# facebookresearch/pytorch3d

Hardware: AMD Instinct MI355X
Metric: rasterized Mpix/s (fwd+bwd) at 512^2 faces_per_pixel=8 (higher is better)
Workload: dtype f32

## Files before the change

### pytorch3d_amd/csrc/raster_mesh.hip

```cpp
#include "binning.h"
#include "tile_map.h"
#include "chunk_order.h"
#include "p3d_geom.h"
#include "topk.h"

#include <stdio.h>
#include <stdlib.h>


namespace p3d {

namespace {

constexpr int kTile = 16;
constexpr int kStage = 256;
constexpr int kMeshPayload = 4;
constexpr int kSplitMaxTiles = 512;

constexpr int kFineWaves = 4;

struct MeshArgs {
  const float* face_verts;
  const int64_t* neighbor;
  const int64_t* mesh_first;
  const int64_t* mesh_count;
  BinCSR csr;
  int N, H, W, K;
  TileMap tm;
  float blur, sqrt_blur;
  int persp, clip, cull;
  int walk_plan;
  int64_t* p2f;
  float* zbuf;
  float* bary;
  float* dists;
  int* cover;
  int CY, CX;
  int* area_count;
  int* area_list;
  int list_by_plan;
  const int* overflow;
  int ties;
  unsigned long long* tie_words;
  int SY, SX;
};

typedef unsigned int u32x4 __attribute__((ext_vector_type(4)));
__device__ __forceinline__ void store16(void* p, unsigned a, unsigned b, unsigned c, unsigned d) {
  u32x4 v = {a, b, c, d};
  *reinterpret_cast<u32x4*>(p) = v;
}

template <int KT>
__device__ __forceinline__ void store_row(float* dst, const float (&v)[KT]) {
  if constexpr (KT % 4 == 0) {
#pragma unroll
    for (int k = 0; k < KT; k += 4) {
      float4 t;
      t.x = v[k];
      t.y = v[k + 1];
      t.z = v[k + 2];
      t.w = v[k + 3];
      *reinterpret_cast<float4*>(dst + k) = t;
    }
  } else if constexpr (KT == 2) {
    float2 t;
    t.x = v[0];
    t.y = v[1];
    *reinterpret_cast<float2*>(dst) = t;
  } else {
#pragma unroll
    for (int k = 0; k < KT; ++k) dst[k] = v[k];
  }
}

template <typename Queue, int KT, bool IN_REGS>
__device__ __forceinline__ void write_pixel(const MeshArgs& a, const Queue& q, int64_t opix) {
  static_assert(IN_REGS, "vector-row stores need the register queue");
  const int64_t base = opix * KT;
  float zv[KT], dv[KT], bv[3 * KT];
  long long iv[KT];
#pragma unroll
  for (int k = 0; k < KT; ++k) {
    const bool ok = q.valid(k);
    iv[k] = ok ? (long long)q.ix(k) : -1ll;
    zv[k] = ok ? q.zf(k) : -1.0f;
    dv[k] = ok ? q.pay(0, k) : -1.0f;
    bv[3 * k + 0] = ok ? q.pay(1, k) : -1.0f;
    bv[3 * k + 1] = ok ? q.pay(2, k) : -1.0f;
    bv[3 * k + 2] = ok ? q.pay(3, k) : -1.0f;
  }
  if constexpr (KT % 4 == 0) {
#pragma unroll
    for (int k = 0; k < KT; k += 4) {
      store16(a.zbuf + base + k, __float_as_uint(zv[k]), __float_as_uint(zv[k + 1]), __float_as_uint(zv[k + 2]),
                  __float_as_uint(zv[k + 3]));
      store16(a.dists + base + k, __float_as_uint(dv[k]), __float_as_uint(dv[k + 1]), __float_as_uint(dv[k + 2]),
                  __float_as_uint(dv[k + 3]));
    }
#pragma unroll
    for (int k = 0; k < 3 * KT; k += 4)
      store16(a.bary + base * 3 + k, __float_as_uint(bv[k]), __float_as_uint(bv[k + 1]), __float_as_uint(bv[k + 2]),
                  __float_as_uint(bv[k + 3]));
#pragma unroll
    for (int k = 0; k < KT; k += 2)
      store16(a.p2f + base + k, (unsigned)iv[k], (unsigned)(iv[k] >> 32), (unsigned)iv[k + 1], (unsigned)(iv[k + 1] >> 32));
  } else {
    store_row<KT>(a.zbuf + base, zv);
    store_row<KT>(a.dists + base, dv);
#pragma unroll
    for (int k = 0; k < 3 * KT; ++k) a.bary[base * 3 + k] = bv[k];
    if constexpr (KT % 2 == 0) {
      long long* ip = reinterpret_cast<long long*>(a.p2f + base);
#pragma unroll
      for (int k = 0; k < KT; k += 2) {
        longlong2 t;
        t.x = iv[k];
        t.y = iv[k + 1];
        *reinterpret_cast<longlong2*>(ip + k) = t;
      }
    } else {
#pragma unroll
      for (int k = 0; k < KT; ++k) a.p2f[base + k] = iv[k];
    }
  }
}

template <typename Queue, int KT, bool IN_REGS>
__device__ __forceinline__ void write_subtile_fill_patch(const MeshArgs& a, const Queue& q, bool have, int n, int sy0,
                                                         int sx0, int y_end, int x_end, int lane, bool pix_ok, int yi,
                                                         int xi) {
  const int H = a.H, W = a.W, K = a.K;
  const int rows = min(8, y_end - sy0), cols = min(8, x_end - sx0);
  const int seg = cols * K;
  const int64_t col0 = W - sx0 - cols;
  const bool patch = have;
  for (int r = 0; r < rows; ++r) {
    const int64_t px = ((int64_t)n * H + (H - 1 - (sy0 + r))) * W + col0;
    if ((K & 3) == 0) {
      const int q4 = seg >> 2;
      const float4 m1 = make_float4(-1.0f, -1.0f, -1.0f, -1.0f);
      longlong2 i1;
      i1.x = -1;
      i1.y = -1;
      float4* zb = reinterpret_cast<float4*>(a.zbuf + px * K);
      float4* db = reinterpret_cast<float4*>(a.dists + px * K);
      float4* bb = reinterpret_cast<float4*>(a.bary + px * K * 3);
      longlong2* ib = reinterpret_cast<longlong2*>(a.p2f + px * K);
      for (int e = lane; e < 3 * q4; e += 64) {
        bb[e] = m1;
        if (e < 2 * q4) ib[e] = i1;
        if (e < q4) {
          zb[e] = m1;
          db[e] = m1;
        }
      }
    } else {
      for (int e = lane; e < 3 * seg; e += 64) {
        a.bary[px * K * 3 + e] = -1.0f;
        if (e < seg) {
          a.p2f[px * K + e] = -1;
// ... 210 lines not shown
    const unsigned alo = (unsigned)__builtin_amdgcn_readlane((int)mlo, ci), ahi = (unsigned)__builtin_amdgcn_readlane((int)mhi, ci);
    unsigned long long inside = ((unsigned long long)ahi << 32) | (unsigned long long)alo;
    float zc = __int_as_float(__builtin_amdgcn_readlane(__float_as_int(zcv), ci));
    if constexpr (!GENERAL) {
      const unsigned long long free_of_a = __ballot(((mlo & alo) | (mhi & ahi)) == 0u) & cand;
      if (free_of_a) {
        const int cb = __builtin_ctzll(free_of_a);
        cand &= ~(1ull << cb);
        const unsigned long long in_b = ((unsigned long long)(unsigned)__builtin_amdgcn_readlane((int)mhi, cb) << 32) |
                                        (unsigned long long)(unsigned)__builtin_amdgcn_readlane((int)mlo, cb);
        const bool mine_is_b = __builtin_amdgcn_inverse_ballot_w64(in_b);
        const int jb = __builtin_amdgcn_readlane(oj, cb);
        const float zb = __int_as_float(__builtin_amdgcn_readlane(__float_as_int(zcv), cb));
        jj = mine_is_b ? jb : jj;
        zc = mine_is_b ? zb : zc;
        inside |= in_b;
      }
    }
    const bool in_box = __builtin_amdgcn_inverse_ballot_w64(inside);
    const bool too_deep = zc > q.kth_z(K);
    if (pix_ok && in_box && !too_deep) {
      const float kz0 = TIES ? q.kth_z(K) : 0.0f;
      const int ki0 = TIES ? q.kth_i(K) : 0;
      if constexpr (TIES && GENERAL) tie_z = INFINITY;
      const float4* rec = reinterpret_cast<const float4*>(reinterpret_cast<const char*>(s_rec) + __umul24((unsigned)jj, (unsigned)(kRecWords * sizeof(float4))));
      const float4 r0 = rec[0], r1 = rec[1], r2 = rec[2];
      const int f = __float_as_int(r2.y);
      FaceHit h;
      bool hit = false;
      {
        const double2 d0 = *reinterpret_cast<const double2*>(&rec[3]);
        const double2 d1 = *reinterpret_cast<const double2*>(&rec[4]);
        FaceRec fr;
        fr.v0 = mk3(r0.x, r0.y, r1.z);
        fr.v1 = mk3(r0.z, r0.w, r1.w);
        fr.v2 = mk3(r1.x, r1.y, r2.x);
        fr.rd_area = d0.x;
        fr.rd_l01 = d0.y;
        fr.rd_l02 = d1.x;
        fr.rd_l12 = d1.y;
        const float4 r5 = rec[5];
        const float2 r6 = *reinterpret_cast<const float2*>(&rec[6]);
        fr.d01 = mk2(r5.x, r5.y);
        fr.d12 = mk2(r5.z, r5.w);
        fr.d20 = mk2(r6.x, r6.y);
        const bool pcs = PC && !GENERAL;
        fr.wide = pcs ? false : __float_as_int(r2.w) != 0;
        const f3 bp = face_depth_rec(fr, p, pcs || persp, pcs || clip, &h);
        const bool adm = !(h.z < 0.0f) & q.admits(K, h.z, f);
        if constexpr (TIES && !GENERAL) {
          const bool ev = (h.z == kz0) & !adm;
          const int d = kz0 == tie_z ? min(tie_drop, f) : f;
          tie_drop = ev ? d : tie_drop;
          tie_z = ev ? kz0 : tie_z;
        }
        if (GENERAL || adm) hit = face_dist_rec<PC && !GENERAL>(fr, p, a.blur, bp, &h);
      }
      if (hit) {
        bool ins = true;
        if constexpr (GENERAL) {
          const int nb = __float_as_int(r2.z);
          if (nb != -1) {
            const int at = q.find(nb);
            if (at >= 0) {
              float queued;
              if constexpr (Queue::kPayload > 0) {
                queued = q.payload_at(0, at);
              } else {
                queued = recompute_face(a, nb, p, persp, clip).dist;
              }
              if (fabsf(h.dist) < fabsf(queued))
                q.erase(at);
              else
                ins = false;
            }
          }
        }
        if (ins && q.admits(K, h.z, f)) {
          if constexpr (Queue::kPayload > 0) {
            const float pl[kMeshPayload] = {h.dist, h.bary.x, h.bary.y, h.bary.z};
            q.insert(K, h.z, f, pl);
          } else {
            const float none[1] = {0.0f};
            q.insert(K, h.z, f, none);
          }
          if constexpr (TIES && !GENERAL) {
            const bool ev = (kz0 < INFINITY) & (q.kth_z(K) == kz0);
            const int d = kz0 == tie_z ? min(tie_drop, ki0) : ki0;
            tie_drop = ev ? d : tie_drop;
            tie_z = ev ? kz0 : tie_z;
          }
        }
      }
    }
  }
}

__device__ __forceinline__ void cover_mark(const MeshArgs& a, int n, int sy0, bool any, int yo, int xo, int lane) {
  unsigned long long rem = __ballot(any);
  const int wid = (yo >> 4) * a.CX + (xo >> 4);
  while (rem) {
    const int w0 = __builtin_amdgcn_readlane(wid, __builtin_ctzll(rem));
    const unsigned long long same = __ballot(any && wid == w0);
    unsigned bits = 0;
#pragma unroll
    for (int j = 0; j < 8; ++j)
      if ((same >> (8 * j)) & 0xffull) bits |= 1u << ((a.H - 1 - (sy0 + j)) & 15);
    rem &= ~same;
    if (lane == 0) {
      const int word = (n * a.CY) * a.CX + w0;
      if (a.area_list != nullptr && !a.list_by_plan) {
        const int before = atomicOr(a.cover + word, (int)bits);
        if (before == 0 && bits != 0u) a.area_list[atomicAdd(a.area_count, 1)] = word;
      } else {
        atomicOr(a.cover + word, (int)bits);
      }
    }
  }
}

__device__ __forceinline__ float uniform_f(float v) { return __int_as_float(__builtin_amdgcn_readfirstlane(__float_as_int(v))); }

struct StageLds {
  unsigned* pm;
  float pxy;
  unsigned valid_c, valid_r;
  float4 (*rec)[kRecWords];
  float* zc;
  int* order;
  float* qlow;
  ChunkOrderScratch* ord;
  int* wcnt;
};

struct TileRect {
  float x0, x1, y0, y1;
};

template <bool BINNED, bool PC = false>
__device__ __forceinline__ int stage_chunk(const MeshArgs& a, const StageLds& l, const TileRect& tile, int64_t src_base,
                                           int count, int base, int tid, bool cull, bool clip, bool prune, bool* general) {
  const int lane = tid & 63, w = tid >> 6;
  const int i = base + tid;
  bool keep = false;
  f3 v0, v1, v2;
  FaceSetup fs;
  int fid = -1, nb = -1;
  unsigned cm = 0, rm = 0;
  const bool has = i < count;
  fs.xlo = fs.xhi = fs.ylo = fs.yhi = 0.0f;
  fs.reject = true;
  if (has) {
    fid = BINNED ? a.csr.list[src_base + i] : (int)(src_base + i);
    const float* g = a.face_verts + (int64_t)fid * 9;
    nb = (int)a.neighbor[fid];
    v0 = mk3(g[0], g[1], g[2]);
    v1 = mk3(g[3], g[4], g[5]);
    v2 = mk3(g[6], g[7], g[8]);
    fs = face_setup(v0, v1, v2, a.sqrt_blur, cull);
  }
  int xb = 0, xa = 0, yb = 0, ya = 0;
  if (__ballot(has) != 0) {
#pragma unroll
    for (int c = 0; c < 16; ++c) {
      const float xs = __int_as_float(__builtin_amdgcn_readlane(__float_as_int(l.pxy), c));
      const float ys = __int_as_float(__builtin_amdgcn_readlane(__float_as_int(l.pxy), 16 + c));
      xb += xs < fs.xlo ? 1 : 0;
      xa += xs > fs.xhi ? 1 : 0;
      yb += ys < fs.ylo ? 1 : 0;
      ya += ys > fs.yhi ? 1 : 0;
    }
  }
  if (has) {
    cm = range_mask16(xb, xa) & l.valid_c;
    rm = range_mask16(yb, ya) & l.valid_r;
    keep = !fs.reject && cm != 0 && rm != 0;
    if (keep && prune)
      keep = !rect_cannot_hit(mk2(v0.x, v0.y), mk2(v1.x, v1.y), mk2(v2.x, v2.y), tile.x0, tile.x1, tile.y0, tile.y1, a.sqrt_blur);
  }
  const unsigned long long km = __ballot(keep);
  if (lane == 0) l.wcnt[w] = __popcll(km);
  __syncthreads();
  int pos = mask_rank(km);
  int staged = 0;
#pragma unroll
  for (int j = 0; j < kStage / kWave; ++j) {
    const int c = l.wcnt[j];
    if (j < w) pos += c;
    staged += c;
  }
  bool gen = false;
  if (keep) {
    FaceRec fr;
    face_rec_make(v0, v1, v2, &fr);
    gen = nb != -1 || (PC && (fr.wide || face_rec_degenerate(fr)));
    l.pm[pos] = cm | (rm << 16);
    l.rec[pos][0] = make_float4(v0.x, v0.y, v1.x, v1.y);
    l.rec[pos][1] = make_float4(v2.x, v2.y, v0.z, v1.z);
    l.rec[pos][2] = make_float4(v2.z, __int_as_float(fid), __int_as_float(nb), __int_as_float(fr.wide ? 1 : 0));
    double2 d0, d1;
    d0.x = fr.rd_area;
    d0.y = fr.rd_l01;
    d1.x = fr.rd_l02;
    d1.y = fr.rd_l12;
    *reinterpret_cast<double2*>(&l.rec[pos][3]) = d0;
    *reinterpret_cast<double2*>(&l.rec[pos][4]) = d1;
    l.rec[pos][5] = make_float4(fr.d01.x, fr.d01.y, fr.d12.x, fr.d12.y);
    l.rec[pos][6] = make_float4(fr.d20.x, fr.d20.y, 0.0f, 0.0f);
    const float zmin = min3(v0.z, v1.z, v2.z);
    l.zc[pos] = (clip && nb == -1 && zmin >= 1e-3f) ? zmin * 0.999998f : -INFINITY;
  }
  *general = __syncthreads_or(gen ? 1 : 0) != 0;
  return staged;
}

struct SubTile {
  float x0, x1, y0, y1;
};

template <bool GENERAL, typename Queue, bool PC = false, bool TIES = false>
__device__ __forceinline__ void wave_chunk(const MeshArgs& a, int K, Queue& q, int staged, bool sorted, const SubTile& st, f2 p,
                                           bool pix_ok, int lane, bool persp, bool clip, bool prune, const unsigned* s_pm,
                                           const float4 (*s_rec)[kRecWords], const float* s_zc, const int* s_order,
                                           const float* s_qlow, int cshift, int rshift, float& tie_z, int& tie_drop, int deal = -1) {
  for (int jb = 0; jb < staged; jb += kWave) {
    const int jfirst = deal >= 0 ? deal * 16 : jb;
    if (jfirst >= staged) break;
    if (sorted && __ballot(pix_ok && !(s_qlow[jfirst] > q.kth_z(K))) == 0) break;
    const int j = deal >= 0 ? (((lane >> 4) * 4 + deal) * 16 + (lane & 15)) : jb + lane;
    bool touch = false;
    int oj = 0;
    unsigned mlo = 0, mhi = 0;
    float zcv = 0.0f;
    if (j < staged) {
      oj = s_order[j];
      const unsigned pm = s_pm[oj];
      const unsigned cmask = (pm >> cshift) & 0xffu, rmask = (pm >> (16 + rshift)) & 0xffu;
      touch = (cmask != 0) & (rmask != 0);
      if (touch && prune) {
        const float4 r0 = s_rec[oj][0], r1 = s_rec[oj][1];
        touch = !rect_cannot_hit(mk2(r0.x, r0.y), mk2(r0.z, r0.w), mk2(r1.x, r1.y), st.x0, st.x1, st.y0, st.y1, a.sqrt_blur);
      }
      block_mask_8x8(cmask, rmask, &mlo, &mhi);
      zcv = s_zc[oj];
    }
    const unsigned long long cand = __ballot(touch);
    eval_candidates<GENERAL, Queue, PC, TIES>(a, K, q, cand, oj, mlo, mhi, zcv, p, pix_ok, persp, clip, s_rec, tie_z, tie_drop);
    if (deal >= 0) break;
  }
}

constexpr int kMergeWords = 2 + kMeshPayload;

template <typename Queue, int KT>
__device__ __forceinline__ void merge_dump(const Queue& q, float* slab, int lane) {
#pragma unroll
  for (int k = 0; k < KT; ++k) {
    slab[(0 * KT + k) * kWave + lane] = q.zf(k);
    slab[(1 * KT + k) * kWave + lane] = __int_as_float(q.ix(k));
#pragma unroll
    for (int pp = 0; pp < kMeshPayload; ++pp) slab[((2 + pp) * KT + k) * kWave + lane] = q.pay(pp, k);
  }
}

template <typename Queue, int KT>
__device__ __forceinline__ void merge_absorb(Queue& q, int K, const float* slab, int lane) {
#pragma unroll 1
  for (int k = 0; k < KT; ++k) {
    const int idx = __float_as_int(slab[(1 * KT + k) * kWave + lane]);
    if (__ballot(idx != kEmptyIdx) == 0) break;
    const float z = slab[(0 * KT + k) * kWave + lane];
    float pl[kMeshPayload];
#pragma unroll
    for (int pp = 0; pp < kMeshPayload; ++pp) pl[pp] = slab[((2 + pp) * KT + k) * kWave + lane];
    if (idx != kEmptyIdx && q.admits(K, z, idx)) q.insert(K, z, idx, pl);
  }
}

template <typename Queue, int KT, bool IN_REGS, bool BINNED, bool EXACT, int WAVES = kFineWaves, bool PC = false,
          bool SPLIT = false, bool TIES = false>
__global__ __launch_bounds__(kStage, WAVES) void mesh_raster_kernel(MeshArgs a) {
  static_assert(!(SPLIT && TIES), "the tie marks of four queues that merge are not tracked: CUDA tie order runs the plain kernels");
  __shared__ float s_merge[SPLIT ? 3 * kMergeWords * KT * kWave : 1];
  __shared__ unsigned s_pm[kStage];
  __shared__ float4 s_rec[kStage][kRecWords];
  __shared__ __align__(16) float s_zc[kStage];
  __shared__ int s_order[kStage];
  __shared__ float s_qlow[kStage];
  __shared__ ChunkOrderScratch s_ord;
  __shared__ int s_wcnt[kStage / kWave];

  if (a.overflow != nullptr && (*a.overflow != 0) == BINNED) return;
  TileCoord tc;
  unsigned blk = SPLIT ? blockIdx.x >> 2 : blockIdx.x;
  bool listed = false;
  if (BINNED && !SPLIT && a.walk_plan && a.csr.plan.hdr[3] != 0) {
    const unsigned A = (unsigned)a.csr.plan.hdr[0], B = (unsigned)a.csr.plan.hdr[1];
    int row;
    if (blk < A) {
      row = a.csr.plan.order[blk];
      if (a.list_by_plan && threadIdx.x == 0) {
        const int per = a.tm.BH * a.tm.BW;
        const int ln = row / per, lrem = row - ln * per, lby = lrem / a.tm.BW, lbx = lrem - lby * a.tm.BW;
        a.area_list[blk] = (ln * a.CY + (a.CY - 1 - lby)) * a.CX + (a.CX - 1 - lbx);
        if (blk == 0) *a.area_count = (int)A;
      }
    } else if (blk < A + B) {
      if (EXACT && (KT & 3) == 0 && A > 0) return;
      row = a.csr.plan.bg_list[blk - A];
    } else {
      return;
    }
    const int per_image = a.tm.BH * a.tm.BW;
    tc.n = row / per_image;
    const int rem = row - tc.n * per_image;
    tc.by = rem / a.tm.BW;
    tc.bx = rem - tc.by * a.tm.BW;
    tc.ty = tc.tx = 0;
    listed = true;
  }
  if (!listed && !tile_of_block(a.tm, blk, &tc)) return;
  const int n = tc.n, by = tc.by, bx = tc.bx, ty = tc.ty, tx = tc.tx;

  const int H = a.H, W = a.W;
  const int y_end = min(H, (by + 1) * a.tm.bin_size);
  const int x_end = min(W, (bx + 1) * a.tm.bin_size);
  const int ty0 = by * a.tm.bin_size + ty * kTile;
  const int tx0 = bx * a.tm.bin_size + tx * kTile;
  if (ty0 >= y_end || tx0 >= x_end) return;

  const int tid = threadIdx.x;
  const int lane = tid & 63;
  const int w = __builtin_amdgcn_readfirstlane(tid >> 6);
  const int sub = SPLIT ? (int)(blockIdx.x & 3u) : w;
  const int sy0 = ty0 + (sub >> 1) * 8;
  const int sx0 = tx0 + (sub & 1) * 8;
  if (SPLIT && (sy0 >= y_end || sx0 >= x_end)) return;
  const int yi = sy0 + (lane >> 3);
  const int xi = sx0 + (lane & 7);
  const bool pix_ok = yi < y_end && xi < x_end;
  const bool wave_ok = sy0 < y_end && sx0 < x_end;

  int64_t src_base;
  int count;
  if (BINNED) {
    const int64_t row = ((int64_t)n * a.tm.BH + by) * a.tm.BW + bx;
    count = a.csr.total[row];
    src_base = a.csr.offset[row];
  } else {
    src_base = a.mesh_first[n];
    count = (int)a.mesh_count[n];
  }
  const bool piggy = BINNED && !SPLIT && EXACT && (KT & 3) == 0 && a.walk_plan != 0 && a.csr.plan.hdr != nullptr;
  int plan_a = 0, plan_b = 0;
  if (piggy) {
    plan_a = a.csr.plan.hdr[0];
    plan_b = a.csr.plan.hdr[1];
  }
  if (BINNED && !SPLIT && a.list_by_plan && !listed && tid == 0) {
    const int64_t row = ((int64_t)n * a.tm.BH + by) * a.tm.BW + bx;
    if (count > 0) a.area_list[a.csr.plan.arank[row]] = (n * a.CY + (a.CY - 1 - by)) * a.CX + (a.CX - 1 - bx);
    if (blockIdx.x == 0) *a.area_count = a.csr.plan.hdr[0];
  }
  if (count <= 0) {
    if (piggy && plan_a > 0) return;
    const int Kbg = EXACT ? KT : a.K;
    if (SPLIT && (Kbg & 3) == 0) {
      fill_tile_background<kStage>(a, n, sy0, sx0, y_end, x_end, tid, 8);
    } else if (SPLIT && w != 0) {
    } else if ((Kbg & 3) == 0) {
      fill_tile_background<kStage>(a, n, ty0, tx0, y_end, x_end, tid);
    } else if constexpr (EXACT && Queue::kPayload > 0) {
      Queue e;
      e.init();
      if (pix_ok) write_pixel<Queue, KT, IN_REGS>(a, e, ((int64_t)n * H + (H - 1 - yi)) * W + (W - 1 - xi));
    } else if (wave_ok) {
      Queue e;
      e.init();
      write_subtile_fill_patch<Queue, KT, IN_REGS>(a, e, false, n, sy0, sx0, y_end, x_end, lane, pix_ok, yi, xi);
    }
    return;
  }

  const int ox = SPLIT ? sx0 : tx0, oy = SPLIT ? sy0 : ty0;
  const float pxy = (lane & 16) ? pix_to_ndc(oy + (lane & 15), H, W) : pix_to_ndc(ox + (lane & 15), W, H);
  auto col_centre = [&](int x) { return __int_as_float(__builtin_amdgcn_readlane(__float_as_int(pxy), x - ox)); };
  auto row_centre = [&](int y) { return __int_as_float(__builtin_amdgcn_readlane(__float_as_int(pxy), 16 + y - oy)); };
  const f2 p = mk2(__int_as_float(__builtin_amdgcn_ds_bpermute((xi - ox) << 2, __float_as_int(pxy))),
                   __int_as_float(__builtin_amdgcn_ds_bpermute((16 + yi - oy) << 2, __float_as_int(pxy))));
  const float tile_x0 = SPLIT ? 0.0f : col_centre(tx0), tile_x1 = SPLIT ? 0.0f : col_centre(min(tx0 + kTile, x_end) - 1);
  const float tile_y0 = SPLIT ? 0.0f : row_centre(ty0), tile_y1 = SPLIT ? 0.0f : row_centre(min(ty0 + kTile, y_end) - 1);
  const float sub_x0 = col_centre(sx0), sub_x1 = col_centre(min(sx0 + 8, x_end) - 1);
  const float sub_y0 = row_centre(sy0), sub_y1 = row_centre(min(sy0 + 8, y_end) - 1);

  Queue q;
  q.init();
  const int K = EXACT ? KT : a.K;
  const bool persp = PC || a.persp != 0, clip = PC || a.clip != 0, cull = a.cull != 0;
  const bool prune = true;
  StageLds lds;
  lds.pm = s_pm;
  {
    const int side = SPLIT ? 8 : kTile;
    const int cols = min(side, x_end - ox), rows = min(side, y_end - oy);
    lds.valid_c = (1u << cols) - 1u;
    lds.valid_r = (1u << rows) - 1u;
    lds.pxy = pxy;
  }
  lds.rec = s_rec;
  lds.zc = s_zc;
  lds.order = s_order;
  lds.qlow = s_qlow;
  lds.ord = &s_ord;
  lds.wcnt = s_wcnt;
  TileRect tile;
  tile.x0 = SPLIT ? sub_x0 : tile_x0;
  tile.x1 = SPLIT ? sub_x1 : tile_x1;
  tile.y0 = SPLIT ? sub_y0 : tile_y0;
  tile.y1 = SPLIT ? sub_y1 : tile_y1;
  SubTile st;
  st.x0 = sub_x0;
  st.x1 = sub_x1;
  st.y0 = sub_y0;
  st.y1 = sub_y1;
  const bool run_waves = wave_ok;

  int base = 0;
  bool general = false;
  float tie_z = -1.0f;
  int tie_drop = kEmptyIdx;
  int staged = 0;
  for (; base < count; base += kStage) {
    staged = stage_chunk<BINNED, PC>(a, lds, tile, src_base, count, base, tid, cull, clip, prune, &general);
    if (general) break;
    chunk_bucket_order(s_zc, staged, s_order, s_qlow, s_ord, tid);
    if (run_waves)
      wave_chunk<false, Queue, PC, TIES>(a, K, q, staged, true, st, p, pix_ok, lane, persp, clip, prune, s_pm, s_rec, s_zc, s_order,
                                         s_qlow, SPLIT ? 0 : (sub & 1) * 8, SPLIT ? 0 : (sub >> 1) * 8, tie_z, tie_drop, SPLIT ? w : -1);
    __syncthreads();
  }
  if constexpr (SPLIT && Queue::kPayload > 0) {
    if (w != 0) merge_dump<Queue, KT>(q, s_merge + (w - 1) * kMergeWords * KT * kWave, lane);
    __syncthreads();
    if (w == 0) {
#pragma unroll 1
      for (int src = 0; src < 3; ++src) merge_absorb<Queue, KT>(q, K, s_merge + src * kMergeWords * KT * kWave, lane);
    }
  }
  if (general) {
    for (;;) {
      if (tid < staged) s_order[tid] = tid;
      __syncthreads();
      if (run_waves && (!SPLIT || w == 0))
        wave_chunk<true, Queue, false, TIES>(a, K, q, staged, false, st, p, pix_ok, lane, persp, clip, prune, s_pm, s_rec, s_zc, s_order,
                                             s_qlow, SPLIT ? 0 : (sub & 1) * 8, SPLIT ? 0 : (sub >> 1) * 8, tie_z, tie_drop);
      __syncthreads();
      base += kStage;
      if (base >= count) break;
      bool dummy = false;
      staged = stage_chunk<BINNED, PC>(a, lds, tile, src_base, count, base, tid, cull, clip, prune, &dummy);
    }
  }

  float tie_kz = 0.0f;
  bool tie_cand = false, tie_gen = false;
  if constexpr (TIES) {
    tie_kz = q.kth_z(K);
    tie_gen = tie_z == INFINITY;
    tie_cand = K > 1 && tie_z == tie_kz && tie_kz < INFINITY;
  }
  {
    if constexpr (Queue::kPayload == 0) {
      static_assert(!SPLIT, "queues without payload do not run in split mode");
      if (wave_ok) write_pixel_long<Queue, KT, EXACT>(a, q, ((int64_t)n * H + (H - 1 - yi)) * W + (W - 1 - xi), p, pix_ok, persp, clip);
      if (a.cover != nullptr && wave_ok) cover_mark(a, n, sy0, pix_ok && q.valid(0), H - 1 - yi, W - 1 - xi, lane);
    } else if constexpr (EXACT) {
      if (pix_ok && (!SPLIT || w == 0)) {
        int l2;
        asm volatile("v_mbcnt_lo_u32_b32 %0, -1, 0\n\tv_mbcnt_hi_u32_b32 %0, -1, %0" : "=v"(l2));
        const int yo = sy0 + (l2 >> 3), xo = sx0 + (l2 & 7);
        write_pixel<Queue, KT, IN_REGS>(a, q, ((int64_t)n * H + (H - 1 - yo)) * W + (W - 1 - xo));
      }
      if (a.cover != nullptr && (!SPLIT || w == 0)) {
        int l2;
        asm volatile("v_mbcnt_lo_u32_b32 %0, -1, 0\n\tv_mbcnt_hi_u32_b32 %0, -1, %0" : "=v"(l2));
        const int yo = sy0 + (l2 >> 3), xo = sx0 + (l2 & 7);
        cover_mark(a, n, sy0, yo < y_end && xo < x_end && q.valid(0), H - 1 - yo, W - 1 - xo, l2);
      }
    } else {
      if (wave_ok) write_subtile_fill_patch<Queue, KT, IN_REGS>(a, q, true, n, sy0, sx0, y_end, x_end, lane, pix_ok, yi, xi);
      if (a.cover != nullptr && wave_ok && (!SPLIT || w == 0)) cover_mark(a, n, sy0, pix_ok && q.valid(0), H - 1 - yi, W - 1 - xi, lane);
    }
  }
  if constexpr (TIES) {
    asm volatile("s_waitcnt vmcnt(0)" ::: "memory");
    int l2;
    asm volatile("v_mbcnt_lo_u32_b32 %0, -1, 0\n\tv_mbcnt_hi_u32_b32 %0, -1, %0" : "=v"(l2));
    const int yo = sy0 + (l2 >> 3), xo = sx0 + (l2 & 7);
    const bool inside = yo < y_end && xo < x_end;
    const int64_t tbase = (((int64_t)n * H + (H - 1 - yo)) * W + (W - 1 - xo)) * K;
    bool tie = tie_gen && inside;
    if (tie_cand && inside) {
      int s_max = -1;
      for (int k = 0; k < K; ++k) {
        const long long fi = __hip_atomic_load(a.p2f + tbase + k, __ATOMIC_RELAXED, __HIP_MEMORY_SCOPE_AGENT);
        const float fz = __int_as_float(__hip_atomic_load(reinterpret_cast<const int*>(a.zbuf + tbase + k), __ATOMIC_RELAXED, __HIP_MEMORY_SCOPE_AGENT));
        if (fi >= 0 && fz < tie_kz) s_max = max(s_max, (int)fi);
      }
      tie = s_max > tie_drop;
    }
    if (tie) a.p2f[tbase] = -2;
    const unsigned long long tmask = __ballot(tie);
    if (a.tie_words != nullptr && wave_ok && l2 == 0) a.tie_words[((int64_t)n * a.SY + (sy0 >> 3)) * a.SX + (sx0 >> 3)] = tmask;
  }
  if constexpr (BINNED && !SPLIT && EXACT && (KT & 3) == 0) {
    if (piggy && plan_b > 0) {
      const int64_t row = ((int64_t)n * a.tm.BH + by) * a.tm.BW + bx;
      const int q_bg = (plan_b + plan_a - 1) / plan_a;
      const long long j0 = (long long)a.csr.plan.arank[row] * q_bg;
      const long long j1 = j0 + q_bg < (long long)plan_b ? j0 + q_bg : (long long)plan_b;
      const int per_image = a.tm.BH * a.tm.BW;
      for (long long j = j0; j < j1; ++j) {
        const int brow = a.csr.plan.bg_list[j];
        const int bn = brow / per_image, brem = brow - bn * per_image;
        const int bby = brem / a.tm.BW, bbx = brem - bby * a.tm.BW;
        const int by_end = min(H, (bby + 1) * a.tm.bin_size), bx_end = min(W, (bbx + 1) * a.tm.bin_size);
        const int bty0 = bby * a.tm.bin_size + ty * kTile, btx0 = bbx * a.tm.bin_size + tx * kTile;
        if (bty0 >= by_end || btx0 >= bx_end) continue;
        if (bty0 + kTile <= by_end && btx0 + kTile <= bx_end)
          fill_tile_full<KT>(a, bn, bty0, btx0, tid);
        else
          fill_tile_background<kStage>(a, bn, bty0, btx0, by_end, bx_end, tid);
      }
    }
  }
}

template <bool BINNED>
__device__ __forceinline__ void replay_pixel(const MeshArgs& a, int n, int yi, int xi, volatile float* qz, volatile int* qi, int lane) {
  const int H = a.H, W = a.W, K = a.K;
  int64_t src;
  int count;
  if (BINNED) {
    const int64_t row = ((int64_t)n * a.tm.BH + yi / a.tm.bin_size) * a.tm.BW + xi / a.tm.bin_size;
    src = a.csr.offset[row];
    count = a.csr.total[row];
  } else {
    src = a.mesh_first[n];
    count = (int)a.mesh_count[n];
  }
  const bool persp = a.persp != 0, clip = a.clip != 0, cull = a.cull != 0;
  auto verts = [&](int f, f3* v0, f3* v1, f3* v2) {
    const float* g = a.face_verts + (int64_t)f * 9;
    *v0 = mk3(g[0], g[1], g[2]);
    *v1 = mk3(g[3], g[4], g[5]);
    *v2 = mk3(g[6], g[7], g[8]);
  };
  struct Batch {
    int f;
    int nb;
    f3 v0, v1, v2;
  };
  auto fetch = [&](int i0) {
    Batch b;
    b.f = -1;
    b.nb = -1;
    b.v0 = b.v1 = b.v2 = mk3(0.0f, 0.0f, 0.0f);
    const int i = i0 + lane;
    if (i < count) {
      b.f = BINNED ? a.csr.list[src + i] : (int)(src + i);
      verts(b.f, &b.v0, &b.v1, &b.v2);
      b.nb = (int)a.neighbor[b.f];
    }
    return b;
  };
  const f2 p = mk2(pix_to_ndc(xi, W, H), pix_to_ndc(yi, H, W));
  const int64_t opix = ((int64_t)n * H + (H - 1 - yi)) * W + (W - 1 - xi);
  int qn = 0, qmax_i = -1;
  float qmax_z = -1000.0f;
  Batch nxt = fetch(0);
  for (int i0 = 0; i0 < count; i0 += kWave) {
    const Batch cur = nxt;
    if (i0 + kWave < count) nxt = fetch(i0 + kWave);
    FaceHit h;
    bool hit = false;
    if (cur.f >= 0) {
      const FaceSetup fs = face_setup(cur.v0, cur.v1, cur.v2, a.sqrt_blur, cull);
      if (!fs.reject && !outside_box(fs, p)) hit = face_hit(cur.v0, cur.v1, cur.v2, p, a.blur, persp, clip, &h);
    }
    unsigned long long hits = __ballot(hit);
    while (hits) {
      const int c = __builtin_ctzll(hits);
      hits &= hits - 1;
      const int cf = __builtin_amdgcn_readlane(cur.f, c);
      const float cz = __int_as_float(__builtin_amdgcn_readlane(__float_as_int(h.z), c));
      const int cnb = __builtin_amdgcn_readlane(cur.nb, c);
      int at = -1;
      if (cnb != -1) {
        for (int j0 = 0; j0 < qn; j0 += kWave) {
          const unsigned long long is = __ballot(j0 + lane < qn && qi[j0 + lane] == cnb);
          if (is) {
            at = j0 + __builtin_ctzll(is);
            break;
          }
        }
      }
      if (at != -1) {
        f3 n0, n1, n2;
        verts(cnb, &n0, &n1, &n2);
        FaceHit hn;
        face_hit(n0, n1, n2, p, a.blur, persp, clip, &hn);
        const float cdist = __int_as_float(__builtin_amdgcn_readlane(__float_as_int(h.dist), c));
        if (fabsf(cdist) < fabsf(hn.dist)) {
          if (lane == 0) {
            qz[at] = cz;
            qi[at] = cf;
          }
          if (cz > qmax_z) {
            qmax_z = cz;
            qmax_i = at;
          }
        }
      } else if (qn < K) {
        if (lane == 0) {
          qz[qn] = cz;
          qi[qn] = cf;
        }
        if (cz > qmax_z) {
          qmax_z = cz;
          qmax_i = qn;
        }
        ++qn;
      } else if (cz < qmax_z) {
        if (lane == 0) {
          qz[qmax_i] = cz;
          qi[qmax_i] = cf;
        }
        qmax_z = cz;
        __builtin_amdgcn_wave_barrier();
        float m = -INFINITY;
        for (int j = lane; j < K; j += kWave) m = fmaxf(m, qz[j]);
        for (int d = 32; d >= 1; d >>= 1) m = fmaxf(m, __shfl_xor(m, d));
        if (m > cz) {
          for (int j0 = 0; j0 < K; j0 += kWave) {
            const unsigned long long is = __ballot(j0 + lane < K && qz[j0 + lane] == m);
            if (is) {
              qmax_i = j0 + __builtin_ctzll(is);
              break;
            }
          }
          qmax_z = m;
        }
      }
      __builtin_amdgcn_wave_barrier();
    }
  }
  for (int j = lane; j < K; j += kWave) {
    const int64_t o = opix * K + j;
    if (j >= qn) {
      a.p2f[o] = -1;
      a.zbuf[o] = a.dists[o] = a.bary[3 * o] = a.bary[3 * o + 1] = a.bary[3 * o + 2] = -1.0f;
    }
  }
  for (int j = lane; j < qn; j += kWave) {
    const float z = qz[j];
    const int f = qi[j];
    int rank = 0;
    for (int t = 0; t < qn; ++t) {
      const float zt = qz[t];
      const int ft = qi[t];
      rank += (zt < z || (zt == z && ft < f)) ? 1 : 0;
    }
    f3 v0, v1, v2;
    verts(f, &v0, &v1, &v2);
    FaceHit h;
    face_hit(v0, v1, v2, p, a.blur, persp, clip, &h);
    const int64_t o = opix * K + rank;
    a.p2f[o] = f;
    a.zbuf[o] = h.z;
    a.dists[o] = h.dist;
    a.bary[3 * o] = h.bary.x;
    a.bary[3 * o + 1] = h.bary.y;
    a.bary[3 * o + 2] = h.bary.z;
  }
  __builtin_amdgcn_wave_barrier();
}

constexpr int kTieWordsPerWave = 16;
// ... 418 lines not shown
```

Baseline: 7348.

## Hoist plan header loads, prefetch background rows, work-steal fills per wave

```diff
diff --git a/profiles/fine_tile_chain.py b/profiles/fine_tile_chain.py
--- /dev/null
+++ b/profiles/fine_tile_chain.py
@@ -0,0 +1,78 @@
+#!/usr/bin/env python
+import argparse
+import ctypes
+import math
+import os
+import sys
+
+import torch
+
+ROOT = os.path.dirname(os.path.dirname(os.path.abspath(__file__)))
+sys.path.insert(0, ROOT)
+sys.path.insert(0, os.path.join(ROOT, "tests"))
+sys.path.insert(0, os.path.join(ROOT, "profiles"))
+
+PHASES = ["entry", "CSR row known (flag, header, order; total, offset)", "list indices arrived", "vertices arrived", "staging published",
+          "order done", "evaluation done", "past the trailing barrier", "pixel stores issued", "background rows known", "exit (fill issued)"]
+
+
+def main():
+    ap = argparse.ArgumentParser()
+    ap.add_argument("lib")
+    ap.add_argument("--iters", type=int, default=5)
+    args = ap.parse_args()
+
+    import _util as U
+    import pytorch3d_amd as p3d
+    from exp_measure import open_lib
+
+    lib = open_lib(os.path.abspath(args.lib))
+    lib.p3d_probe_chain_read.restype = None
+    lib.p3d_probe_chain_read.argtypes = [ctypes.POINTER(ctypes.c_ulonglong)]
+    d = torch.device("cuda:0")
+    B, H, K = 64, 512, 8
+    blur = math.log(1.0 / 1e-4 - 1.0) * 1e-4
+    verts, faces = U.hetero_batch(B, seed=0, torus_div=1.0)
+    m = p3d.PackedMeshes([v.to(d) for v in verts], [f.to(d) for f in faces])
+    fv = m.verts_packed()[m.faces_packed()].contiguous()
+    F = int(fv.shape[0])
+    first, count = m.mesh_to_faces_packed_first_idx().contiguous(), m.num_faces_per_mesh().contiguous()
+    nbr = torch.full((F,), -1, dtype=torch.int64, device=d)
+    bin_size, M = 32, int(max(10000, F / 5))
+    out = (torch.empty((B, H, H, K), dtype=torch.int64, device=d), torch.empty((B, H, H, K), device=d),
+           torch.empty((B, H, H, K, 3), device=d), torch.empty((B, H, H, K), device=d))
+    cover = torch.empty((B, H // 16, H // 16), dtype=torch.int32, device=d)
+    ws = torch.empty((int(lib.p3d_rasterize_meshes_workspace_bytes(F, B, H, H, bin_size, M)),), dtype=torch.uint8, device=d)
+    stream = ctypes.c_void_p(torch.cuda.current_stream(d).cuda_stream)
+
+    def run():
+        rc = lib.p3d_rasterize_meshes_ex(fv.data_ptr(), first.data_ptr(), count.data_ptr(), nbr.data_ptr(), F, B, H, H, blur, K, bin_size, M,
+                                         1, 1, 0, out[0].data_ptr(), out[1].data_ptr(), out[2].data_ptr(), out[3].data_ptr(),
+                                         cover.data_ptr(), 0, ws.data_ptr(), ws.numel(), stream)
+        assert rc == 0, rc
+
+    buf = (ctypes.c_ulonglong * 32)()
+    run()
+    torch.cuda.synchronize()
+    lib.p3d_probe_chain_read(buf)
+    for _ in range(args.iters):
+        run()
+    torch.cuda.synchronize()
+    lib.p3d_probe_chain_read(buf)
+    v = list(buf)
+    waves, ticks = v[31], v[15]
+    cyc = sum(v[1:11])
+    if waves == 0 or ticks == 0:
+        raise SystemExit("the probe counted nothing: is this a -DP3D_PROBE_CHAIN library?")
+    mhz = cyc / ticks * 100.0
+    print(f"probed waves {waves} ({args.iters} launches), mean life {cyc / waves:.0f} shader clocks = {ticks / waves / 100.0:.2f} us "
+          f"(shader clock {mhz:.0f} MHz)")
+    print(f"{'phase (time since the point before)':<52}{'waves':>9}{'clocks':>10}{'us':>8}{'share':>8}")
+    for i in range(1, 11):
+        n = v[16 + i]
+        mean = v[i] / n if n else 0.0
+        print(f"{PHASES[i]:<52}{n:>9}{mean:>10.0f}{mean / mhz:>8.2f}{100.0 * v[i] / cyc:>7.1f}%")
+
+
+if __name__ == "__main__":
+    main()
diff --git a/pytorch3d_amd/csrc/raster_mesh.hip b/pytorch3d_amd/csrc/raster_mesh.hip
--- a/pytorch3d_amd/csrc/raster_mesh.hip
+++ b/pytorch3d_amd/csrc/raster_mesh.hip
@@ -7,6 +7,63 @@
 #include <stdio.h>
 #include <stdlib.h>
 
+
+#ifdef P3D_PROBE_CHAIN
+__device__ unsigned long long g_chain[32];
+extern "C" __attribute__((visibility("default"))) void p3d_probe_chain_read(unsigned long long* out) {
+  (void)hipDeviceSynchronize();
+  (void)hipMemcpyFromSymbol(out, HIP_SYMBOL(g_chain), sizeof(unsigned long long) * 32);
+  unsigned long long z[32] = {0};
+  (void)hipMemcpyToSymbol(HIP_SYMBOL(g_chain), z, sizeof(z));
+}
+namespace p3d {
+namespace {
+constexpr int kChainStamps = 11;
+__shared__ unsigned long long s_chain[4][kChainStamps + 1];
+__device__ __forceinline__ void chain_note(int i, unsigned long long t) {
+  if ((threadIdx.x & 63) == 0) s_chain[threadIdx.x >> 6][i] = t;
+}
+__device__ __forceinline__ void chain_stamp(int i) { chain_note(i, __builtin_readcyclecounter()); }
+__device__ __forceinline__ void chain_flush(unsigned long long r0) {
+  const int lane = threadIdx.x & 63, w = threadIdx.x >> 6;
+  if (s_chain[w][kChainStamps] == 0ull || lane >= kChainStamps) return;
+  if (lane == 0) {
+    atomicAdd(&g_chain[15], (unsigned long long)__builtin_amdgcn_s_memrealtime() - r0);
+    atomicAdd(&g_chain[31], 1ull);
+    return;
+  }
+  const unsigned long long t1 = s_chain[w][lane];
+  int prev = lane - 1;
+  while (prev > 0 && s_chain[w][prev] == 0ull) --prev;
+  if (t1 == 0ull) return;
+  atomicAdd(&g_chain[lane], t1 - s_chain[w][prev]);
+  atomicAdd(&g_chain[16 + lane], 1ull);
+}
+}
+}
+#define P3D_CHAIN_ENTRY()                                                                                        \
+  const unsigned long long chain_t0 = __builtin_readcyclecounter();                                              \
+  const unsigned long long chain_r0 = __builtin_amdgcn_s_memrealtime();                                          \
+  if ((threadIdx.x & 63) < kChainStamps + 1) s_chain[threadIdx.x >> 6][threadIdx.x & 63] = 0ull
+#define P3D_CHAIN_ARM(on)                                                                 \
+  if ((on) && (blockIdx.x & 7u) == 0u) {                                                  \
+    chain_note(kChainStamps, 1ull);                                                       \
+    chain_note(0, chain_t0);                                                              \
+  }
+#define P3D_CHAIN_STAMP(i) chain_stamp(i)
+#define P3D_CHAIN_ARRIVED(i, ...)               \
+  do {                                          \
+    asm volatile("" ::__VA_ARGS__ : "memory");  \
+    chain_stamp(i);                             \
+  } while (0)
+#define P3D_CHAIN_FLUSH() chain_flush(chain_r0)
+#else
+#define P3D_CHAIN_ENTRY() ((void)0)
+#define P3D_CHAIN_ARM(on) ((void)0)
+#define P3D_CHAIN_STAMP(i) ((void)0)
+#define P3D_CHAIN_ARRIVED(i, ...) ((void)0)
+#define P3D_CHAIN_FLUSH() ((void)0)
+#endif
 
 namespace p3d {
 
@@ -523,11 +580,13 @@
   fs.reject = true;
   if (has) {
     fid = BINNED ? a.csr.list[src_base + i] : (int)(src_base + i);
+    P3D_CHAIN_ARRIVED(2, "v"(fid));
     const float* g = a.face_verts + (int64_t)fid * 9;
     nb = (int)a.neighbor[fid];
     v0 = mk3(g[0], g[1], g[2]);
     v1 = mk3(g[3], g[4], g[5]);
     v2 = mk3(g[6], g[7], g[8]);
+    P3D_CHAIN_ARRIVED(3, "v"(v0.x), "v"(v1.y), "v"(v2.z), "v"(nb));
     fs = face_setup(v0, v1, v2, a.sqrt_blur, cull);
   }
   int xb = 0, xa = 0, yb = 0, ya = 0;
@@ -660,22 +719,29 @@
   __shared__ float s_qlow[kStage];
   __shared__ ChunkOrderScratch s_ord;
   __shared__ int s_wcnt[kStage / kWave];
-
+  __shared__ int s_fill_ticket;
+
+  P3D_CHAIN_ENTRY();
+  __builtin_amdgcn_s_setprio(3);
+  unsigned blk = SPLIT ? blockIdx.x >> 2 : blockIdx.x;
+  const bool plan_walk = BINNED && !SPLIT && a.walk_plan != 0;
+  int hdr_a = 0, hdr_b = 0, hdr_order = 0;
+  int walk_row = 0;
+  if (plan_walk) {
+    hdr_a = a.csr.plan.hdr[0];
+    hdr_b = a.csr.plan.hdr[1];
+    hdr_order = a.csr.plan.hdr[3];
+    const unsigned rows = (unsigned)(a.N * a.tm.BH * a.tm.BW);
+    walk_row = a.csr.plan.order[blk < rows ? blk : rows - 1u];
+  }
   if (a.overflow != nullptr && (*a.overflow != 0) == BINNED) return;
   TileCoord tc;
-  unsigned blk = SPLIT ? blockIdx.x >> 2 : blockIdx.x;
   bool listed = false;
-  if (BINNED && !SPLIT && a.walk_plan && a.csr.plan.hdr[3] != 0) {
-    const unsigned A = (unsigned)a.csr.plan.hdr[0], B = (unsigned)a.csr.plan.hdr[1];
+  if (plan_walk && hdr_order != 0) {
+    const unsigned A = (unsigned)hdr_a, B = (unsigned)hdr_b;
     int row;
     if (blk < A) {
-      row = a.csr.plan.order[blk];
-      if (a.list_by_plan && threadIdx.x == 0) {
-        const int per = a.tm.BH * a.tm.BW;
-        const int ln = row / per, lrem = row - ln * per, lby = lrem / a.tm.BW, lbx = lrem - lby * a.tm.BW;
-        a.area_list[blk] = (ln * a.CY + (a.CY - 1 - lby)) * a.CX + (a.CX - 1 - lbx);
-        if (blk == 0) *a.area_count = (int)A;
-      }
+      row = walk_row;
     } else if (blk < A + B) {
       if (EXACT && (KT & 3) == 0 && A > 0) return;
       row = a.csr.plan.bg_list[blk - A];
@@ -688,6 +754,10 @@
     tc.by = rem / a.tm.BW;
     tc.bx = rem - tc.by * a.tm.BW;
     tc.ty = tc.tx = 0;
+    if (blk < A && a.list_by_plan && threadIdx.x == 0) {
+      a.area_list[blk] = (tc.n * a.CY + (a.CY - 1 - tc.by)) * a.CX + (a.CX - 1 - tc.bx);
+      if (blk == 0) *a.area_count = (int)A;
+    }
     listed = true;
   }
   if (!listed && !tile_of_block(a.tm, blk, &tc)) return;
@@ -712,27 +782,37 @@
   const bool pix_ok = yi < y_end && xi < x_end;
   const bool wave_ok = sy0 < y_end && sx0 < x_end;
 
+  const bool piggy = BINNED && !SPLIT && EXACT && (KT & 3) == 0 && plan_walk;
   int64_t src_base;
   int count;
+  int fill_slot = (int)blk;
   if (BINNED) {
     const int64_t row = ((int64_t)n * a.tm.BH + by) * a.tm.BW + bx;
     count = a.csr.total[row];
     src_base = a.csr.offset[row];
+    if (!listed && (piggy || (!SPLIT && a.list_by_plan))) fill_slot = a.csr.plan.arank[row];
   } else {
     src_base = a.mesh_first[n];
     count = (int)a.mesh_count[n];
   }
-  const bool piggy = BINNED && !SPLIT && EXACT && (KT & 3) == 0 && a.walk_plan != 0 && a.csr.plan.hdr != nullptr;
-  int plan_a = 0, plan_b = 0;
-  if (piggy) {
-    plan_a = a.csr.plan.hdr[0];
-    plan_b = a.csr.plan.hdr[1];
-  }
+  const int plan_a = piggy ? hdr_a : 0, plan_b = piggy ? hdr_b : 0;
+  int bg_n = 0, bg_row0 = 0, bg_row1 = 0;
+  long long bg_j0 = 0;
+  if (piggy && plan_b > 0 && count > 0) {
+    const int q_bg = (plan_b + plan_a - 1) / plan_a;
+    bg_j0 = (long long)fill_slot * q_bg;
+    const long long left = (long long)plan_b - bg_j0;
+    bg_n = left < 0 ? 0 : (left < q_bg ? (int)left : q_bg);
+    if (bg_n > 0) bg_row0 = a.csr.plan.bg_list[bg_j0];
+    if (bg_n > 1) bg_row1 = a.csr.plan.bg_list[bg_j0 + 1];
+  }
+  if (tid == 0) s_fill_ticket = 0;
   if (BINNED && !SPLIT && a.list_by_plan && !listed && tid == 0) {
-    const int64_t row = ((int64_t)n * a.tm.BH + by) * a.tm.BW + bx;
-    if (count > 0) a.area_list[a.csr.plan.arank[row]] = (n * a.CY + (a.CY - 1 - by)) * a.CX + (a.CX - 1 - bx);
-    if (blockIdx.x == 0) *a.area_count = a.csr.plan.hdr[0];
-  }
+    if (count > 0) a.area_list[fill_slot] = (n * a.CY + (a.CY - 1 - by)) * a.CX + (a.CX - 1 - bx);
+    if (blockIdx.x == 0) *a.area_count = hdr_a;
+  }
+  P3D_CHAIN_ARM(BINNED && listed && count > 0 && count <= kStage);
+  P3D_CHAIN_STAMP(1);
   if (count <= 0) {
     if (piggy && plan_a > 0) return;
     const int Kbg = EXACT ? KT : a.K;
@@ -804,12 +884,18 @@
   for (; base < count; base += kStage) {
     staged = stage_chunk<BINNED, PC>(a, lds, tile, src_base, count, base, tid, cull, clip, prune, &general);
     if (general) break;
+    P3D_CHAIN_STAMP(4);
     chunk_bucket_order(s_zc, staged, s_order, s_qlow, s_ord, tid);
+    P3D_CHAIN_STAMP(5);
+    __builtin_amdgcn_s_setprio(0);
     if (run_waves)
       wave_chunk<false, Queue, PC, TIES>(a, K, q, staged, true, st, p, pix_ok, lane, persp, clip, prune, s_pm, s_rec, s_zc, s_order,
                                          s_qlow, SPLIT ? 0 : (sub & 1) * 8, SPLIT ? 0 : (sub >> 1) * 8, tie_z, tie_drop, SPLIT ? w : -1);
-    __syncthreads();
-  }
+    P3D_CHAIN_STAMP(6);
+    if (base + kStage < count) __syncthreads();
+    P3D_CHAIN_STAMP(7);
+  }
+  __builtin_amdgcn_s_setprio(0);
   if constexpr (SPLIT && Queue::kPayload > 0) {
     if (w != 0) merge_dump<Queue, KT>(q, s_merge + (w - 1) * kMergeWords * KT * kWave, lane);
     __syncthreads();
@@ -884,27 +970,35 @@
     const unsigned long long tmask = __ballot(tie);
     if (a.tie_words != nullptr && wave_ok && l2 == 0) a.tie_words[((int64_t)n * a.SY + (sy0 >> 3)) * a.SX + (sx0 >> 3)] = tmask;
   }
+  P3D_CHAIN_STAMP(8);
   if constexpr (BINNED && !SPLIT && EXACT && (KT & 3) == 0) {
-    if (piggy && plan_b > 0) {
-      const int64_t row = ((int64_t)n * a.tm.BH + by) * a.tm.BW + bx;
-      const int q_bg = (plan_b + plan_a - 1) / plan_a;
-      const long long j0 = (long long)a.csr.plan.arank[row] * q_bg;
-      const long long j1 = j0 + q_bg < (long long)plan_b ? j0 + q_bg : (long long)plan_b;
+    if (bg_n > 0) {
+      P3D_CHAIN_ARRIVED(9, "s"(bg_row0), "s"(bg_row1));
+      int l2;
+      asm volatile("v_mbcnt_lo_u32_b32 %0, -1, 0\n\tv_mbcnt_hi_u32_b32 %0, -1, %0" : "=v"(l2));
       const int per_image = a.tm.BH * a.tm.BW;
-      for (long long j = j0; j < j1; ++j) {
-        const int brow = a.csr.plan.bg_list[j];
+      for (;;) {
+        int t = 0;
+        if (l2 == 0) t = atomicAdd(&s_fill_ticket, 1);
+        t = __builtin_amdgcn_readfirstlane(t);
+        const int j = t >> 2;
+        if (j >= bg_n) break;
+        const int brow = j == 0 ? bg_row0 : (j == 1 ? bg_row1 : a.csr.plan.bg_list[bg_j0 + j]);
+        const int vtid = (t & 3) * kWave + l2;
         const int bn = brow / per_image, brem = brow - bn * per_image;
         const int bby = brem / a.tm.BW, bbx = brem - bby * a.tm.BW;
         const int by_end = min(H, (bby + 1) * a.tm.bin_size), bx_end = min(W, (bbx + 1) * a.tm.bin_size);
         const int bty0 = bby * a.tm.bin_size + ty * kTile, btx0 = bbx * a.tm.bin_size + tx * kTile;
         if (bty0 >= by_end || btx0 >= bx_end) continue;
         if (bty0 + kTile <= by_end && btx0 + kTile <= bx_end)
-          fill_tile_full<KT>(a, bn, bty0, btx0, tid);
+          fill_tile_full<KT>(a, bn, bty0, btx0, vtid);
         else
-          fill_tile_background<kStage>(a, bn, bty0, btx0, by_end, bx_end, tid);
-      }
-    }
-  }
+          fill_tile_background<kStage>(a, bn, bty0, btx0, by_end, bx_end, vtid);
+      }
+    }
+  }
+  P3D_CHAIN_STAMP(10);
+  P3D_CHAIN_FLUSH();
 }
 
 template <bool BINNED>
```

Result: faster. 7851, median of 6 (+6.8%).
